# j4n1k/rl4co-slap

Measured on AMD Instinct MI355X. Metric: env-steps/sec (batch×decode) SLAP & TSP-100 at 1/2/4/8 MI355X, higher is better.
Workload: dtype u8+i64+f32

## Files before the change

rl4co_slap_amd/csrc/co_common.hpp:

```cpp
#pragma once

#include <hip/hip_runtime.h>
#include <stdint.h>

#include "../../include/co_env.h"

namespace co {

constexpr int kWave = 64;

__device__ __forceinline__ int lane_id() { return threadIdx.x & (kWave - 1); }
__device__ __forceinline__ int wave_in_block() {
  return __builtin_amdgcn_readfirstlane(threadIdx.x >> 6);
}

template <typename T>
__device__ __forceinline__ T wave_sum(T v) {
#pragma unroll
  for (int off = 32; off > 0; off >>= 1) v += __shfl_xor(v, off, kWave);
  return v;
}

__device__ __forceinline__ float wave_max(float v) {
#pragma unroll
  for (int off = 32; off > 0; off >>= 1) v = fmaxf(v, __shfl_xor(v, off, kWave));
  return v;
}

__device__ __forceinline__ int wave_min_int(int v) {
#pragma unroll
  for (int off = 32; off > 0; off >>= 1) v = min(v, __shfl_xor(v, off, kWave));
  return v;
}

__device__ __forceinline__ bool argmax_better(float a, int ia, float b, int ib) {
  const bool na = a != a, nb = b != b;
  if (na || nb) return na && (!nb || ia < ib);
  return a > b || (a == b && ia < ib);
}

__device__ __forceinline__ void wave_argmax(float& v, int& idx) {
#pragma unroll
  for (int off = 32; off > 0; off >>= 1) {
    const float ov = __shfl_xor(v, off, kWave);
    const int oi = __shfl_xor(idx, off, kWave);
    if (argmax_better(ov, oi, v, idx)) { v = ov; idx = oi; }
  }
}

__device__ __forceinline__ void wave_argmin(float& v, int& idx) {
#pragma unroll
  for (int off = 32; off > 0; off >>= 1) {
    const float ov = __shfl_xor(v, off, kWave);
    const int oi = __shfl_xor(idx, off, kWave);
    if (ov < v || (ov == v && oi < idx)) { v = ov; idx = oi; }
  }
}

__device__ __forceinline__ void set_status(int32_t* status, int32_t bits) {
  if (status) atomicOr(status, bits);
}

__device__ __forceinline__ float edge_len(float x0, float y0, float x1, float y1) {
  const float dx = x1 - x0, dy = y1 - y0;
  return sqrtf(dx * dx + dy * dy);
}

template <int CTRL>
__device__ __forceinline__ uint32_t dpp_u(uint32_t v) {
  return (uint32_t)__builtin_amdgcn_update_dpp(0, (int)v, CTRL, 0xf, 0xf, false);
}

template <int RL, class Take>
__device__ __forceinline__ void grp_reduce2(uint32_t& v, uint32_t& a, Take take) {
  uint32_t ov, oa;
#define CO_DPP_STAGE(C)                      \
  ov = dpp_u<C>(v);                          \
  oa = dpp_u<C>(a);                          \
  if (take(ov, oa, v, a)) { v = ov; a = oa; }
  if (RL >= 2) { CO_DPP_STAGE(0xB1); }
  if (RL >= 4) { CO_DPP_STAGE(0x4E); }
  if (RL >= 8) { CO_DPP_STAGE(0x141); }
  if (RL >= 16) { CO_DPP_STAGE(0x140); }
#undef CO_DPP_STAGE
  if (RL >= 32) {
    const auto rv = __builtin_amdgcn_permlane16_swap(v, v, false, false);
    const auto ra = __builtin_amdgcn_permlane16_swap(a, a, false, false);
    v = rv[0]; a = ra[0];
    if (take(rv[1], ra[1], v, a)) { v = rv[1]; a = ra[1]; }
  }
  if (RL >= 64) {
    const auto rv = __builtin_amdgcn_permlane32_swap(v, v, false, false);
    const auto ra = __builtin_amdgcn_permlane32_swap(a, a, false, false);
    v = rv[0]; a = ra[0];
    if (take(rv[1], ra[1], v, a)) { v = rv[1]; a = ra[1]; }
  }
}

template <int RL, class Op>
__device__ __forceinline__ uint32_t grp_reduce(uint32_t v, Op op) {
  if (RL >= 2) v = op(v, dpp_u<0xB1>(v));
  if (RL >= 4) v = op(v, dpp_u<0x4E>(v));
  if (RL >= 8) v = op(v, dpp_u<0x141>(v));
  if (RL >= 16) v = op(v, dpp_u<0x140>(v));
  if (RL >= 32) {
    const auto r = __builtin_amdgcn_permlane16_swap(v, v, false, false);
    v = op(r[0], r[1]);
  }
  if (RL >= 64) {
    const auto r = __builtin_amdgcn_permlane32_swap(v, v, false, false);
    v = op(r[0], r[1]);
  }
  return v;
}

template <int RL>
__device__ __forceinline__ double grp_sum_f64(double v) {
  uint32_t lo = (uint32_t)__double_as_longlong(v), hi = (uint32_t)(__double_as_longlong(v) >> 32);
  auto join = [](uint32_t l, uint32_t h) {
    return __longlong_as_double((long long)(((uint64_t)h << 32) | l));
  };
#define CO_DPP_F64(C)                                   \
  {                                                     \
    v = v + join(dpp_u<C>(lo), dpp_u<C>(hi));           \
    lo = (uint32_t)__double_as_longlong(v);             \
    hi = (uint32_t)(__double_as_longlong(v) >> 32);     \
  }
  if (RL >= 2) CO_DPP_F64(0xB1);
  if (RL >= 4) CO_DPP_F64(0x4E);
  if (RL >= 8) CO_DPP_F64(0x141);
  if (RL >= 16) CO_DPP_F64(0x140);
#undef CO_DPP_F64
  if (RL >= 32) {
    const auto rl = __builtin_amdgcn_permlane16_swap(lo, lo, false, false);
    const auto rh = __builtin_amdgcn_permlane16_swap(hi, hi, false, false);
    v = join(rl[0], rh[0]) + join(rl[1], rh[1]);
    lo = (uint32_t)__double_as_longlong(v);
    hi = (uint32_t)(__double_as_longlong(v) >> 32);
  }
  if (RL >= 64) {
    const auto rl = __builtin_amdgcn_permlane32_swap(lo, lo, false, false);
    const auto rh = __builtin_amdgcn_permlane32_swap(hi, hi, false, false);
    v = join(rl[0], rh[0]) + join(rl[1], rh[1]);
  }
  return v;
}

template <int RL>
__device__ __forceinline__ float grp_max(float v) {
  return __uint_as_float(grp_reduce<RL>(__float_as_uint(v), [](uint32_t x, uint32_t y) {
    return __float_as_uint(fmaxf(__uint_as_float(x), __uint_as_float(y)));
  }));
}
template <int RL>
__device__ __forceinline__ float grp_max_ord(float v) {
  const int b = __float_as_int(v);
  int o = b ^ ((b >> 31) & 0x7fffffff);
  o = (int)grp_reduce<RL>((uint32_t)o, [](uint32_t x, uint32_t y) {
    return (uint32_t)max((int)x, (int)y);
  });
  return __int_as_float(o ^ ((o >> 31) & 0x7fffffff));
}
template <int RL>
__device__ __forceinline__ float grp_sum(float v) {
  return __uint_as_float(grp_reduce<RL>(__float_as_uint(v), [](uint32_t x, uint32_t y) {
    return __float_as_uint(__uint_as_float(x) + __uint_as_float(y));
  }));
}
template <int RL>
__device__ __forceinline__ void grp_argmax(float& v, int& idx) {
  uint32_t uv = __float_as_uint(v), ui = (uint32_t)idx;
  grp_reduce2<RL>(uv, ui, [](uint32_t ov, uint32_t oi, uint32_t cv, uint32_t ci) {
    return argmax_better(__uint_as_float(ov), (int)oi, __uint_as_float(cv), (int)ci);
  });
  v = __uint_as_float(uv);
  idx = (int)ui;
}
template <int RL>
__device__ __forceinline__ int grp_min_int(int v) {
  return (int)grp_reduce<RL>((uint32_t)v, [](uint32_t x, uint32_t y) {
    return (uint32_t)min((int)x, (int)y);
  });
}
template <int RL>
__device__ __forceinline__ int grp_max_int(int v) {
  return (int)grp_reduce<RL>((uint32_t)v, [](uint32_t x, uint32_t y) {
    return (uint32_t)max((int)x, (int)y);
  });
}

template <int RL>
__device__ __forceinline__ void grp_argmin(float& v, int& idx) {
  uint32_t uv = __float_as_uint(v), ui = (uint32_t)idx;
  grp_reduce2<RL>(uv, ui, [](uint32_t ov, uint32_t oi, uint32_t cv, uint32_t ci) {
    const float a = __uint_as_float(ov), b = __uint_as_float(cv);
    return a < b || (a == b && (int)oi < (int)ci);
  });
  v = __uint_as_float(uv);
  idx = (int)ui;
}

template <int RL>
__device__ __forceinline__ void grp_argmin_split(float& v, int& idx) {
  const float m = __uint_as_float(grp_reduce<RL>(__float_as_uint(v), [](uint32_t a, uint32_t b) {
    return __float_as_uint(fminf(__uint_as_float(a), __uint_as_float(b)));
  }));
  const int cand = v == m ? idx : 0x7fffffff;
  idx = (int)grp_reduce<RL>((uint32_t)cand, [](uint32_t a, uint32_t b) {
    return (uint32_t)min((int)a, (int)b);
  });
  v = m;
}

constexpr uint32_t kDistKeyInf = 0xff800000u;
__device__ __forceinline__ uint32_t dist_key(float d) {
  const uint32_t u = __float_as_uint(d + 0.0f);
  return u ^ ((uint32_t)((int32_t)u >> 31) | 0x80000000u);
}
__device__ __forceinline__ uint32_t key_sel32(uint64_t m, uint32_t t, uint32_t f) {
  uint32_t r;
  asm("v_cndmask_b32_e64 %0, %1, %2, %3" : "=v"(r) : "v"(f), "v"(t), "s"(m));
  return r;
}
__device__ __forceinline__ void key_cswap(uint64_t& a, uint64_t& b) {
  const uint64_t lt = __builtin_amdgcn_ballot_w64(a < b);
  const uint32_t alo = (uint32_t)a, ahi = (uint32_t)(a >> 32), blo = (uint32_t)b,
                 bhi = (uint32_t)(b >> 32);
  a = ((uint64_t)key_sel32(lt, ahi, bhi) << 32) | key_sel32(lt, alo, blo);
  b = ((uint64_t)key_sel32(lt, bhi, ahi) << 32) | key_sel32(lt, blo, alo);
}
template <int E>
__device__ __forceinline__ void sort_keys(uint64_t (&k)[E]) {
  static_assert((E & (E - 1)) == 0, "E must be a power of two");
#pragma unroll
  for (int p = 1; p < E; p <<= 1)
#pragma unroll
    for (int q = p; q > 0; q >>= 1)
#pragma unroll
      for (int j = q % p; j + q < E; j += 2 * q)
#pragma unroll
        for (int i = 0; i < q; ++i)
          if (i + j + q < E && (i + j) / (2 * p) == (i + j + q) / (2 * p))
            key_cswap(k[i + j], k[i + j + q]);
}

typedef __attribute__((address_space(3))) void lds_void;

template <int AUX = 0>
__device__ __forceinline__ void stage_bytes_lds(const unsigned char* __restrict__ src, int nbytes,
                                                unsigned char* dst) {
  const int lane = threadIdx.x & 63, wave = wave_in_block(), nw = blockDim.x >> 6;
  const int n16 = nbytes & ~15;
  for (int base = wave * 1024; base < n16; base += nw * 1024) {
    const int off = base + lane * 16;
    if (off < n16)
      __builtin_amdgcn_global_load_lds((const void*)(src + off), (lds_void*)(dst + base), 16, 0,
                                       AUX);
  }
  for (int k = n16 + (int)threadIdx.x; k < nbytes; k += blockDim.x) dst[k] = src[k];
  __builtin_amdgcn_s_waitcnt(0);
  __syncthreads();
}

template <int AUX = 0>
__device__ __forceinline__ void wave_dma(const unsigned char* __restrict__ src, int nbytes,
                                         unsigned char* dst) {
  const int lane = lane_id(), n16 = nbytes & ~15;
  for (int base = 0; base < n16; base += 1024) {
    if (base + lane * 16 < n16)
      __builtin_amdgcn_global_load_lds((const void*)(src + base + lane * 16),
                                       (lds_void*)(dst + base), 16, 0, AUX);
  }
  if (lane < ((nbytes - n16) >> 2))
    reinterpret_cast<uint32_t*>(dst + n16)[lane] = reinterpret_cast<const uint32_t*>(src + n16)[lane];
}

__device__ __forceinline__ void wave_dma_wait() {
  __builtin_amdgcn_s_waitcnt(0);
  __builtin_amdgcn_fence(__ATOMIC_RELEASE, "wavefront");
  __builtin_amdgcn_wave_barrier();
  __builtin_amdgcn_fence(__ATOMIC_ACQUIRE, "wavefront");
}

namespace {
__global__ void zero_i32_kernel(int32_t* p) { *p = 0; }
}
inline int zero_i32(int32_t* p, hipStream_t s) {
  hipLaunchKernelGGL(zero_i32_kernel, dim3(1), dim3(1), 0, s, p);
  return (int)hipGetLastError();
}

inline unsigned grid_for(int64_t work_items, int per_block, int64_t cap = 256 * 16) {
  int64_t g = (work_items + per_block - 1) / per_block;
  if (g < 1) g = 1;
  if (g > cap) g = cap;
  return (unsigned)g;
}

constexpr int64_t kMaxCoverThreads = ((int64_t)1 << 32) - 1;
inline unsigned cover_grid(int64_t work_items, int per_block, int block_threads = 256) {
  int64_t g = (work_items + per_block - 1) / per_block;
  if (g < 1) g = 1;
  if (g * (int64_t)block_threads > kMaxCoverThreads) return 0;
  return (unsigned)g;
}

inline int launch_status() {
  hipError_t e = hipGetLastError();
  return e == hipSuccess ? CO_OK : (int)e;
}

}

int co_internal_tsp_reward_stepmajor(int64_t B, int64_t N, const float* locs,
                                     int64_t locs_batch, const int64_t* acts, int64_t st,
                                     int check, float* reward, int32_t* status, void* stream);
int co_internal_tsp_reward_rows(int64_t B, int64_t N, const float* locs, int64_t locs_batch,
                                const int64_t* acts, int64_t sb, int check, float* reward,
                                int32_t* status, void* stream);
int co_internal_tsp_nearest_rollout(int64_t B, int64_t N, const float* locs, int64_t* acts_out,
                                    uint8_t* mask_out, int64_t* first_out, int64_t* cur_out,
                                    int64_t* i_out, uint8_t* done_out, uint8_t* step_reward_out,
                                    float* reward_out, void* stream);
```

rl4co_slap_amd/csrc/rollout.hip:

```cpp
#include "co_common.hpp"

using namespace co;

namespace {


inline int NW_launch(int64_t n) {
  const int w = (int)((n + 63) / 64);
  return w <= 1 ? 1 : (w == 2 ? 2 : 4);
}

template <int NW>
__device__ __forceinline__ void mask_row_to_lds(const uint64_t (&m)[NW], int n,
                                                unsigned char* row, int c_lo = 0,
                                                int c_hi = -1) {
  if (c_hi < 0) c_hi = n;
  if ((n & 3) == 0 && (c_lo & 3) == 0) {
    for (int c = c_lo; c < c_hi; c += 4) {
      uint32_t v = 0;
#pragma unroll
      for (int j = 0; j < 4; ++j) {
        const int cc = c + j;
        uint64_t w = 0;
#pragma unroll
        for (int k = 0; k < NW; ++k)
          if ((cc >> 6) == k) w = m[k];
        v |= (uint32_t)((w >> (cc & 63)) & 1ull) << (8 * j);
      }
      *reinterpret_cast<uint32_t*>(row + c) = v;
    }
  } else {
    for (int c = c_lo; c < c_hi; ++c) {
      uint64_t w = 0;
#pragma unroll
      for (int k = 0; k < NW; ++k)
        if ((c >> 6) == k) w = m[k];
      row[c] = (unsigned char)((w >> (c & 63)) & 1ull);
    }
  }
}

__device__ __forceinline__ void copy_tile_out(const unsigned char* scratch, int nbytes,
                                              uint8_t* __restrict__ dst) {
  const int tid = threadIdx.x;
  const int n16 = ((reinterpret_cast<uintptr_t>(dst) & 15) == 0) ? (nbytes & ~15) : 0;
  for (int off = tid * 16; off < n16; off += blockDim.x * 16)
    *reinterpret_cast<uint4*>(dst + off) = *reinterpret_cast<const uint4*>(scratch + off);
  for (int k = n16 + tid; k < nbytes; k += blockDim.x) dst[k] = scratch[k];
}

__device__ __forceinline__ void zero_tile_out(int nbytes, uint8_t* __restrict__ dst) {
  const int tid = threadIdx.x;
  const int n16 = ((reinterpret_cast<uintptr_t>(dst) & 15) == 0) ? (nbytes & ~15) : 0;
  for (int off = tid * 16; off < n16; off += blockDim.x * 16)
    *reinterpret_cast<uint4*>(dst + off) = make_uint4(0u, 0u, 0u, 0u);
  for (int k = n16 + tid; k < nbytes; k += blockDim.x) dst[k] = 0;
}

__host__ __device__ inline size_t tsp_tile_bytes(int N, int Q) {
  const size_t xy = (size_t)64 * N * 8;
  const size_t scr = (((size_t)64 * N + 15) & ~(size_t)15) + (size_t)Q * 64 * 8 + 64 * 8 + 64 * 4 +
                     16 * 4;
  return ((xy > scr ? xy : scr) + 15) & ~(size_t)15;
}

#ifndef CO_TEACH_Q
#define CO_TEACH_Q 4
#endif
#ifndef CO_TEACH_U
#define CO_TEACH_U 8
#endif
template <int NW, int Q, bool STATE, int NB = 0>
__global__ __launch_bounds__(64 * Q) void tsp_teacher_kernel(
    int64_t B, int N, const float2* __restrict__ locs, int64_t LB,
    const int64_t* __restrict__ acts_in, uint8_t* __restrict__ mask_out,
    int64_t* __restrict__ first_out, int64_t* __restrict__ cur_out, int64_t* __restrict__ i_out,
    uint8_t* __restrict__ done_out, uint8_t* __restrict__ step_reward_out,
    float* __restrict__ reward_out, int check, int32_t* status) {
  extern __shared__ __attribute__((aligned(16))) unsigned char smem[];
  float2* s_xy = reinterpret_cast<float2*>(smem);
  constexpr int VS = 2 * NW + 1;
  uint32_t* s_vis = reinterpret_cast<uint32_t*>(smem + tsp_tile_bytes(N, Q));
  const int lane = threadIdx.x & 63, q = wave_in_block();
  const int64_t row0 = (int64_t)blockIdx.x * 64;
  const int rows = (int)((B - row0) < 64 ? (B - row0) : 64);
  const int64_t b = row0 + lane;
  const bool live = lane < rows;

  const int R = (N - 1 + Q - 1) / Q;
  const int t_lo = 1 + q * R < N ? 1 + q * R : N;
  const int t_hi = t_lo + R < N ? t_lo + R : N;
  constexpr int U = CO_TEACH_U;
  int64_t bufA[U], bufB[U];
  const int64_t* ap = acts_in + (live ? b : row0);
  auto load = [&](int64_t (&dst)[U], int t0) {
    const int tc = t0 + U <= t_hi ? t0 : t_hi - U;
    const int64_t* p = ap + (int64_t)tc * B;
#pragma unroll
    for (int u = 0; u < U; ++u) {
      dst[u] = *p;
      p += B;
    }
  };
  const int nfull = (t_hi - t_lo) / U;
  const int64_t a_prev = ap[(int64_t)(q == 0 ? 0 : t_lo - 1) * B];
  if (nfull > 0) load(bufA, t_lo);
  if (q == 0) {
    for (int k = 0; k < NW; ++k) {
      const int lo = k * 64;
      const uint64_t w = (N >= lo + 64) ? ~0ull : (N > lo ? ((1ull << (N - lo)) - 1ull) : 0ull);
      s_vis[lane * VS + 2 * k] = (uint32_t)w;
      s_vis[lane * VS + 2 * k + 1] = (uint32_t)(w >> 32);
    }
  }
  stage_bytes_lds(reinterpret_cast<const unsigned char*>(locs + (row0 % LB) * N), rows * N * 8,
                  reinterpret_cast<unsigned char*>(s_xy));
  const float2* xy = s_xy + lane * N;
  uint32_t* vw = s_vis + lane * VS;
  uint32_t badw = 0;
  int a = 0;
  float px = 0.f, py = 0.f, fx = 0.f, fy = 0.f;
  double len = 0.0;
  if (live) {
    const uint32_t lo = (uint32_t)a_prev;
    const uint32_t in = ((uint32_t)(a_prev >> 32) == 0u) & (lo < (uint32_t)N);
    a = in ? (int)lo : 0;
    if (q == 0) {
      badw |= in ^ 1u;
      __hip_atomic_fetch_and(&vw[a >> 5], ~(1u << (a & 31)), __ATOMIC_RELAXED,
                             __HIP_MEMORY_SCOPE_WORKGROUP);
    }
    const float2 p0 = xy[a];
    px = fx = p0.x;
    py = fy = p0.y;
    auto run = [&](const int64_t (&src)[U], int cnt) {
      int av[U];
#pragma unroll
      for (int u = 0; u < U; ++u) {
        if (u < cnt) {
          const uint32_t l32 = (uint32_t)src[u];
          const uint32_t ok = ((uint32_t)(src[u] >> 32) == 0u) & (l32 < (uint32_t)N);
          badw |= ok ^ 1u;
          av[u] = ok ? (int)l32 : 0;
        }
      }
      float2 qq[U];
#pragma unroll
      for (int u = 0; u < U; ++u)
        if (u < cnt) qq[u] = xy[av[u]];
#pragma unroll
      for (int u = 0; u < U; ++u)
        if (u < cnt)
          __hip_atomic_fetch_and(&vw[av[u] >> 5], ~(1u << (av[u] & 31)), __ATOMIC_RELAXED,
                                 __HIP_MEMORY_SCOPE_WORKGROUP);
      __builtin_amdgcn_sched_barrier(0);
#pragma unroll
      for (int u = 0; u < U; ++u) {
        if (u < cnt) {
          const float ox = u ? qq[u - 1].x : px, oy = u ? qq[u - 1].y : py;
          const float dx = qq[u].x - ox, dy = qq[u].y - oy;
          len += (double)__builtin_amdgcn_sqrtf(dx * dx + dy * dy);
        }
      }
#pragma unroll
      for (int u = 0; u < U; ++u)
        if (u + 1 == cnt) {
          px = qq[u].x;
          py = qq[u].y;
          a = av[u];
        }
    };
    int k = 0;
    for (; k + 1 < nfull; k += 2) {
      load(bufB, t_lo + (k + 1) * U);
      run(bufA, U);
      load(bufA, t_lo + (k + 2) * U);
      run(bufB, U);
    }
    if (k < nfull) run(bufA, U);
    const int tail = t_hi - t_lo - nfull * U;
    if (tail > 0) {
      const int t0 = t_lo + nfull * U;
#pragma unroll
      for (int u = 0; u < U; ++u) bufB[u] = (u < tail) ? ap[(int64_t)(t0 + u) * B] : 0;
      run(bufB, tail);
    }
  }
  if (__any(badw != 0u && check) && lane == 0) set_status(status, CO_ST_INVALID_TOUR);
  __syncthreads();
  const int qlast = N >= 2 ? (N - 2) / R : 0;
  const size_t mbytes = ((size_t)64 * N + 15) & ~(size_t)15;
  double* s_len = reinterpret_cast<double*>(smem + mbytes);
  float2* s_last = reinterpret_cast<float2*>(s_len + Q * 64);
  int* s_lasta = reinterpret_cast<int*>(s_last + 64);
  s_len[q * 64 + lane] = len;
  if (q == qlast) {
    s_last[lane] = make_float2(px, py);
    s_lasta[lane] = a;
  }
  uint64_t m[NW];
#pragma unroll
  for (int kk = 0; kk < NW; ++kk) m[kk] = (uint64_t)vw[2 * kk] | ((uint64_t)vw[2 * kk + 1] << 32);
  bool empty = true;
#pragma unroll
  for (int kk = 0; kk < NW; ++kk) empty &= (m[kk] == 0);
  if (q == 0 && __any(live && !empty && check) && lane == 0)
    set_status(status, CO_ST_INVALID_TOUR);
  int* s_flag = s_lasta + 64;
  bool all_empty = false;
  if (STATE) {
    const bool wave_empty = __ballot(live && !empty) == 0ull;
    if (lane == 0) s_flag[q] = wave_empty;
    __syncthreads();
    all_empty = true;
#pragma unroll
    for (int w = 0; w < Q; ++w) all_empty &= s_flag[w] != 0;
  }
  if (STATE && !all_empty) {
    if (live) {
      const int per = ((N + 4 * Q - 1) / (4 * Q)) * 4;
      const int c_lo = q * per < N ? q * per : N;
      const int c_hi = c_lo + per < N ? c_lo + per : N;
      mask_row_to_lds<NW>(m, N, smem + (size_t)lane * N, c_lo, c_hi);
    }
    __syncthreads();
  } else if (!STATE) {
    __syncthreads();
  }
  if (q == 0 && live) {
    double tot = 0.0;
#pragma unroll
    for (int w = 0; w < Q; ++w) tot += s_len[w * 64 + lane];
    const float2 pl = s_last[lane];
    const int first = ((uint64_t)a_prev < (uint64_t)N) ? (int)a_prev : 0;
    tot += (double)edge_len(pl.x, pl.y, fx, fy);
    reward_out[b] = -(float)tot;
    if (STATE) {
      first_out[b] = first;
      cur_out[b] = s_lasta[lane];
      i_out[b] = N;
      done_out[b] = empty;
      step_reward_out[b] = 0;
    }
  }
  if (STATE) {
    if (all_empty)
      zero_tile_out(rows * N, mask_out + row0 * N);
    else
      copy_tile_out(smem, rows * N, mask_out + row0 * N);
  }
}

#ifndef CO_ROWS_EPL112
#define CO_ROWS_EPL112 7
#endif

__host__ __device__ inline size_t tsp_rows_wave_bytes(int gpw, int N) {
  return ((size_t)gpw * N * 8 + 15) & ~(size_t)15;
}

#ifndef CO_ROWS_WPB
#define CO_ROWS_WPB 4
#endif
template <int G, int EPL, int MODE, bool STATE>
__global__ __launch_bounds__(64 * CO_ROWS_WPB) void tsp_teacher_rows_kernel(
    int64_t B, int N, const float2* __restrict__ locs, int64_t LB,
    const int64_t* __restrict__ acts, int64_t sb, uint8_t* __restrict__ mask_out,
    int64_t* __restrict__ first_out, int64_t* __restrict__ cur_out, int64_t* __restrict__ i_out,
    uint8_t* __restrict__ done_out, uint8_t* __restrict__ step_reward_out,
    float* __restrict__ reward_out, int check, int32_t* status) {
  constexpr int GPW = 64 / G;
  constexpr bool VEC = MODE == 1 && EPL % 2 == 0, DMA = MODE == 3;
  __shared__ uint32_t s_bits[CO_ROWS_WPB][GPW][(G * EPL + 31) / 32];
  extern __shared__ __attribute__((aligned(16))) unsigned char s_rows[];
  constexpr int NWB = (G * EPL + 31) / 32;
  const int lane = lane_id(), sl = lane % G, grp = lane / G, w = wave_in_block();
  uint32_t* bits = s_bits[w][grp];
  unsigned char* s_w = s_rows + (DMA ? (size_t)w * tsp_rows_wave_bytes(GPW, N) : 0);
  const float2* s_xy = reinterpret_cast<const float2*>(s_w);
  const int64_t wid = (int64_t)blockIdx.x * (blockDim.x >> 6) + w;
  const int nwords = (N + 31) >> 5;
  const int t0 = sl * EPL;
  {
    const int64_t base = wid * GPW;
    if (base >= B) return;
    const int64_t r = base + grp;
    const bool valid = r < B;
    const int64_t rr = valid ? r : 0;
    const int64_t* arow = acts + rr * sb;
    if constexpr (DMA) {
      __builtin_amdgcn_s_waitcnt(0xc07f);
      const int rows = (int)(B - base < GPW ? B - base : GPW);
      const int64_t lb = LB == B ? base : base % LB;
      wave_dma<2>(reinterpret_cast<const unsigned char*>(locs + lb * N), rows * N * 8, s_w);
    }
    int64_t av[EPL];
    if constexpr (MODE == 3) {
#pragma unroll
      for (int k = 0; k < EPL; ++k) av[k] = arow[t0 + k < N ? t0 + k : N - 1];
    }
    if constexpr (DMA) wave_dma_wait();
    if constexpr (MODE == 3) {
    } else if constexpr (VEC) {
#pragma unroll
      for (int k = 0; k < EPL; k += 2) {
        if (valid && t0 + k + 1 < N) {
          const longlong2 v = *reinterpret_cast<const longlong2*>(arow + t0 + k);
          av[k] = v.x;
          av[k + 1] = v.y;
        } else {
          av[k] = (valid && t0 + k < N) ? arow[t0 + k] : 0;
          av[k + 1] = 0;
        }
      }
    } else {
#pragma unroll
      for (int k = 0; k < EPL; ++k) av[k] = (valid && t0 + k < N) ? arow[t0 + k] : 0;
    }
    for (int j = sl; j < NWB; j += G) bits[j] = 0u;
    uint32_t bad = 0;
    int node[EPL];
#pragma unroll
    for (int k = 0; k < EPL; ++k) {
      const uint32_t l32 = (uint32_t)av[k];
      const bool ok = ((uint32_t)(av[k] >> 32) == 0u) & (l32 < (uint32_t)N);
      const bool in = t0 + k < N;
      bad |= (in && !ok) ? 1u : 0u;
      node[k] = ok ? (int)l32 : 0;
    }
    const float2* lrow = DMA ? s_xy + grp * N : locs + (LB == B ? rr : rr % LB) * (int64_t)N;
    float2 p[EPL];
    if constexpr (DMA) {
#pragma unroll
      for (int k = 0; k < EPL; ++k) p[k] = lrow[node[k]];
    } else {
#pragma unroll
      for (int k = 0; k < EPL; ++k)
        p[k] = (valid && t0 + k < N) ? lrow[node[k]] : make_float2(0.f, 0.f);
    }
    __builtin_amdgcn_fence(__ATOMIC_RELEASE, "wavefront");
    __builtin_amdgcn_wave_barrier();
    __builtin_amdgcn_fence(__ATOMIC_ACQUIRE, "wavefront");
#pragma unroll
    for (int k = 0; k < EPL; ++k)
      __hip_atomic_fetch_or(&bits[node[k] >> 5],
                            (valid && t0 + k < N) ? 1u << (node[k] & 31) : 0u, __ATOMIC_RELAXED,
                            __HIP_MEMORY_SCOPE_WAVEFRONT);
    double acc = 0.0;
#pragma unroll
    for (int k = 1; k < EPL; ++k) {
      const float dx = p[k].x - p[k - 1].x, dy = p[k].y - p[k - 1].y;
      const float e = __builtin_amdgcn_sqrtf(dx * dx + dy * dy);
      acc += t0 + k < N ? (double)e : 0.0;
    }
    const float nx = __shfl_down(p[0].x, 1, G), ny = __shfl_down(p[0].y, 1, G);
    const float fx = __shfl(p[0].x, 0, G), fy = __shfl(p[0].y, 0, G);
    const int tl = N - 1 - t0;
    float lx = p[EPL - 1].x, ly = p[EPL - 1].y;
#pragma unroll
    for (int k = 0; k < EPL - 1; ++k)
      if (k == tl) {
        lx = p[k].x;
        ly = p[k].y;
      }
    {
      const bool cross = t0 + EPL < N, closing = !cross && tl >= 0 && tl < EPL;
      const float tx = cross ? nx : fx, ty = cross ? ny : fy;
      const float dx = tx - lx, dy = ty - ly;
      const float e = __builtin_amdgcn_sqrtf(dx * dx + dy * dy);
      acc += (cross || closing) ? (double)e : 0.0;
    }
    const float len = (float)grp_sum_f64<G>(acc);
    __builtin_amdgcn_fence(__ATOMIC_RELEASE, "wavefront");
    __builtin_amdgcn_wave_barrier();
    __builtin_amdgcn_fence(__ATOMIC_ACQUIRE, "wavefront");
    int cnt = 0;
    for (int j = sl; j < nwords; j += G) cnt += __popc(bits[j]);
    cnt = (int)grp_reduce<G>((uint32_t)cnt, [](uint32_t x, uint32_t y) { return x + y; });
    bad = grp_reduce<G>(bad, [](uint32_t x, uint32_t y) { return x | y; });
    const bool full = cnt == N;
    if (check && valid && sl == 0 && (bad || !full)) set_status(status, CO_ST_INVALID_TOUR);
    if (!valid) return;
    if constexpr (STATE) {
      uint8_t* mrow = mask_out + r * (int64_t)N;
      const bool wide = ((reinterpret_cast<uintptr_t>(mrow) | (uintptr_t)N) & 3) == 0;
      if (wide) {
        for (int c4 = sl; c4 < (N >> 2); c4 += G) {
          uint32_t v = 0;
          if (!full) {
            const uint32_t nib = ~(bits[c4 >> 3] >> (4 * (c4 & 7))) & 0xfu;
            v = (nib & 1u) | ((nib & 2u) << 7) | ((nib & 4u) << 14) | ((nib & 8u) << 21);
          }
          __builtin_nontemporal_store(v, reinterpret_cast<uint32_t*>(mrow + 4 * c4));
        }
      } else {
        for (int c = sl; c < N; c += G)
          mrow[c] = full ? 0 : (uint8_t)(((bits[c >> 5] >> (c & 31)) & 1u) ^ 1u);
      }
      const int last_lane = (N - 1) / EPL;
      int lastnode = node[0];
#pragma unroll
      for (int k = 0; k < EPL; ++k)
        if (k == tl) lastnode = node[k];
      if (sl == 0) {
        first_out[r] = node[0];
        i_out[r] = N;
        reward_out[r] = -(float)len;
      }
      if (sl == last_lane) cur_out[r] = lastnode;
      if (sl == (G > 2 ? 2 : 1) % G) {
        done_out[r] = full;
        step_reward_out[r] = 0;
      }
    } else {
      if (sl == 0) reward_out[r] = -(float)len;
    }
  }
}

__device__ __forceinline__ float edge_len_hw(float x0, float y0, float x1, float y1) {
  const float dx = x1 - x0, dy = y1 - y0;
  return __builtin_amdgcn_sqrtf(dx * dx + dy * dy);
}
__device__ __forceinline__ int slap_pick_loc(int pp, const int32_t* asg, int L, bool& range) {
  const bool neg = pp < 0;
  int64_t loc = asg[neg ? 0 : pp];
  loc = loc < 0 ? loc + L : loc;
  const bool bad = neg || loc < 0 || loc >= L;
  range |= bad;
  return bad ? 0 : (int)loc;
}
template <int KU, typename PK>
__device__ __forceinline__ float slap_order_len(const PK* pk, const int32_t* asg,
                                                const float2* xy, int L, bool& range,
                                                int K = KU) {
  int pp[KU], lc[KU];
  float2 q[KU];
#pragma unroll
  for (int k = 0; k < KU; ++k) pp[k] = k < K ? pk[k] : 0;
#pragma unroll
  for (int k = 0; k < KU; ++k) lc[k] = k < K ? slap_pick_loc(pp[k], asg, L, range) : 0;
#pragma unroll
  for (int k = 0; k < KU; ++k) q[k] = xy[lc[k]];
  float len = 0.f;
#pragma unroll
  for (int k = 1; k < KU; ++k)
    if (k < K) len += edge_len_hw(q[k - 1].x, q[k - 1].y, q[k].x, q[k].y);
  float2 ql = q[0];
#pragma unroll
  for (int k = 1; k < KU; ++k) ql = (k == K - 1) ? q[k] : ql;
  return len + edge_len_hw(ql.x, ql.y, q[0].x, q[0].y);
}

__host__ __device__ inline size_t slap_asg_bytes(int ipb, int P) {
  return ((size_t)ipb * P * 4 + 15) & ~(size_t)15;
}
__host__ __device__ inline size_t slap_wave_bytes(int gpw, int epl, int L, int O, int K) {
  const size_t keys = (size_t)epl * 64 * 8;
  const size_t data = (size_t)gpw * (L * 8 + O * 4 + O * K * 2);
  return ((keys > data ? keys : data) + 15) & ~(size_t)15;
}
__host__ __device__ inline size_t slap_xy_bytes(int gpw, int L) {
  return ((size_t)gpw * L * 8 + 15) & ~(size_t)15;
}
__host__ __device__ inline size_t slap_wave_bytes_sd(int gpw, int epl, int L, int O, int K) {
  size_t area = (size_t)(epl - 2) * 64 * 8;
  const size_t dd = (size_t)gpw * L * 4, tail = (size_t)gpw * (O * 4 + O * K * 2);
  area = area > dd ? area : dd;
  area = area > tail ? area : tail;
  return slap_xy_bytes(gpw, L) + ((area + 15) & ~(size_t)15);
}

__device__ __forceinline__ float2 ld_pair(const float2* p) { return *p; }

template <int G, int EPL, bool CLOSEST, bool SD>
__global__ __launch_bounds__(256) void slap_group_kernel(
    int64_t B, int L, int P, int O, int K, const float2* __restrict__ locs,
    const int64_t* __restrict__ picklist, const float* __restrict__ depot_dist,
    const int32_t* __restrict__ assign_in, const int64_t* __restrict__ acts_in,
    int64_t* __restrict__ acts_out, uint8_t* __restrict__ mask_out,
    int32_t* __restrict__ assign_out, int64_t* __restrict__ i_out, uint8_t* __restrict__ done_out,
    uint8_t* __restrict__ step_reward_out, float* __restrict__ reward_out,
    float* __restrict__ ratio_out, int32_t* status) {
  constexpr int IPB = 256 / G, GPW = 64 / G;
  extern __shared__ __attribute__((aligned(16))) unsigned char smem[];
  const int lane = lane_id(), sl = lane % G, g = threadIdx.x / G, gw = lane / G;
  int32_t* s_asg = reinterpret_cast<int32_t*>(smem);
  unsigned char* wreg =
      smem + slap_asg_bytes(IPB, P) +
      (size_t)wave_in_block() * (SD ? slap_wave_bytes_sd(GPW, EPL, L, O, K)
                                    : slap_wave_bytes(GPW, EPL, L, O, K));
  unsigned char* area = wreg + (SD ? slap_xy_bytes(GPW, L) : 0);
  uint64_t* s_keys = reinterpret_cast<uint64_t*>(area) - (SD ? 2 * 64 : 0);
  const int64_t b = (int64_t)blockIdx.x * IPB + g;
  const bool live = b < B;
  const int64_t bb = live ? b : 0;
  float2* xy = reinterpret_cast<float2*>(wreg) + gw * L;
  int32_t* asg = s_asg + g * P;
  unsigned char* obase = SD ? area : wreg + (size_t)GPW * L * 8;
  float* olen = reinterpret_cast<float*>(obase) + gw * O;
  int16_t* pks = reinterpret_cast<int16_t*>(obase + (size_t)GPW * O * 4) + gw * O * K;
  const int64_t wbase = (int64_t)blockIdx.x * IPB + (int64_t)wave_in_block() * GPW;
  const int wrows = (int)(B - wbase < GPW ? (B - wbase > 0 ? B - wbase : 0) : GPW);
  if constexpr (SD) {
    wave_dma<2>(reinterpret_cast<const unsigned char*>(depot_dist + wbase * L), wrows * L * 4,
                area);
    wave_dma_wait();
  }

  float dd[EPL];
  uint32_t avail = 0;
#pragma unroll
  for (int k = 0; k < EPL; ++k) {
    const int c = sl + G * k;
    const bool ok = c < L && c != 0;
    if (ok) avail |= 1u << k;
    if constexpr (SD)
      dd[k] = (CLOSEST && ok) ? reinterpret_cast<const float*>(area)[gw * L + c] : __builtin_inff();
    else
      dd[k] = (CLOSEST && ok) ? (depot_dist + bb * L)[c] : __builtin_inff();
  }
  if constexpr (SD) {
    __builtin_amdgcn_s_waitcnt(0xc07f);
    wave_dma<2>(reinterpret_cast<const unsigned char*>(locs + wbase * L), wrows * L * 8, wreg);
  }
  if (live && ratio_out) {
    float* rrow = ratio_out + bb * L;
    if (((reinterpret_cast<uintptr_t>(ratio_out) | ((uintptr_t)L * 4)) & 15) == 0) {
      for (int c4 = sl; c4 < (L >> 2); c4 += G)
        *reinterpret_cast<float4*>(rrow + 4 * c4) = make_float4(0.f, 0.f, 0.f, 0.f);
    } else {
      for (int c = sl; c < L; c += G) rrow[c] = 0.f;
    }
  }
  const float2* lrow = locs + bb * L;
  const int64_t* prow = picklist + bb * (int64_t)O * K;
  float2 xr[EPL];
  int64_t pr[EPL];
#pragma unroll
  for (int k = 0; k < EPL; ++k) {
    const int c = sl + G * k;
    if constexpr (!SD) xr[k] = c < L ? ld_pair(lrow + c) : make_float2(0.f, 0.f);
    pr[k] = c < O * K ? prow[c] : 0;
  }
  auto wrap_product = [&](int64_t pp) -> int32_t {
    if (pp < 0) pp += P;
    return (pp < 0 || pp >= P) ? -1 : (int32_t)pp;
  };
  int32_t pw[EPL];
#pragma unroll
  for (int k = 0; k < EPL; ++k) pw[k] = wrap_product(pr[k]);
  uint64_t key[EPL];
  if (CLOSEST) {
#pragma unroll
    for (int k = 0; k < EPL; ++k)
      key[k] = ((uint64_t)dist_key(dd[k]) << 32) | (uint32_t)(sl + G * k);
    sort_keys<EPL>(key);
  }
  bool range = false;
  if (CLOSEST) {
    uint64_t hk = key[0], nk = EPL > 1 ? key[1] : ~0ull;
#pragma unroll
    for (int k = 2; k < EPL; ++k) s_keys[k * 64 + lane] = key[k];
    int h = 2;
    for (int t = 0; t < P; ++t) {
      const uint32_t hh = (uint32_t)(hk >> 32);
      const uint32_t gm = grp_reduce<G>(hh, [](uint32_t x, uint32_t y) { return x < y ? x : y; });
      const uint32_t cand = hh == gm ? (uint32_t)hk : 0xffffffffu;
      const uint32_t gi =
          grp_reduce<G>(cand, [](uint32_t x, uint32_t y) { return x < y ? x : y; });
      const bool any = gm < kDistKeyInf;
      if (any && (uint32_t)hk == gi) {
        avail &= ~(1u << (gi / G));
        hk = nk;
        nk = h < EPL ? s_keys[h * 64 + lane] : ~0ull;
        ++h;
      }
      if (sl == 0) asg[t] = any ? (int32_t)gi : 0;
    }
  } else {
    int32_t* s_w = reinterpret_cast<int32_t*>(wreg) + gw * P;
    if (P * GPW <= EPL * 128) {
#pragma unroll 4
      for (int t = sl; t < P; t += G) {
        const int64_t a64 = acts_in[(int64_t)t * B + bb];
        asg[t] = (int32_t)a64;
        const int64_t a = a64 < 0 ? a64 + L : a64;
        const bool bad = a < 0 || a >= L;
        range |= bad;
        s_w[t] = bad ? -1 : (int)a;
      }
      __builtin_amdgcn_fence(__ATOMIC_RELEASE, "wavefront");
      __builtin_amdgcn_wave_barrier();
      __builtin_amdgcn_fence(__ATOMIC_ACQUIRE, "wavefront");
      for (int t = 0; t < P; ++t) {
        const int a = s_w[t];
        if (a >= 0 && sl == a % G) avail &= ~(1u << (a / G));
      }
    } else {
      for (int t = 0; t < P; ++t) {
        const int64_t a64 = acts_in[(int64_t)t * B + bb];
        if (sl == 0) asg[t] = (int32_t)a64;
        const int64_t a = a64 < 0 ? a64 + L : a64;
        if (a < 0 || a >= L) {
          range = true;
        } else if (sl == (int)(a % G)) {
          avail &= ~(1u << (int)(a / G));
        }
      }
    }
  }
  if constexpr (SD) {
    __builtin_amdgcn_s_waitcnt(0);
  } else {
#pragma unroll
    for (int k = 0; k < EPL; ++k) {
      const int c = sl + G * k;
      if (c < L) xy[c] = xr[k];
    }
  }
#pragma unroll
  for (int k = 0; k < EPL; ++k) {
    const int c = sl + G * k;
    if (c < O * K) pks[c] = (int16_t)pw[k];
  }
  for (int c = sl + G * EPL; c < O * K; c += G) pks[c] = (int16_t)wrap_product(prow[c]);
  __builtin_amdgcn_fence(__ATOMIC_RELEASE, "wavefront");
  __builtin_amdgcn_wave_barrier();
  __builtin_amdgcn_fence(__ATOMIC_ACQUIRE, "wavefront");

  if (CLOSEST) {
    constexpr int IPW = 64 / G;
    const int w0 = wave_in_block() * IPW;
    for (int idx = lane; idx < IPW * P; idx += 64) {
      const int t = idx / IPW, gi = idx - t * IPW;
      const int64_t be = (int64_t)blockIdx.x * IPB + w0 + gi;
      if (be < B) {
        int64_t* dst = acts_out + (int64_t)t * B + be;
        *dst = (int64_t)s_asg[(w0 + gi) * P + t];
      }
    }
  }
  for (int o = sl; o < O; o += G) {
    const int16_t* pk = pks + o * K;
    float len = 0.f;
    if (K == 5) {
      len = slap_order_len<5>(pk, asg, xy, L, range);
    } else if (K <= 8) {
      len = slap_order_len<8>(pk, asg, xy, L, range, K);
    } else {
      float2 p0 = make_float2(0.f, 0.f), prev = p0;
      for (int k = 0; k < K; ++k) {
        const float2 q = xy[slap_pick_loc(pk[k], asg, L, range)];
        if (k == 0) {
          p0 = q;
        } else {
          len += edge_len_hw(prev.x, prev.y, q.x, q.y);
        }
        prev = q;
      }
      len += edge_len_hw(prev.x, prev.y, p0.x, p0.y);
    }
    olen[o] = len;
  }
  __builtin_amdgcn_fence(__ATOMIC_RELEASE, "wavefront");
  __builtin_amdgcn_wave_barrier();
  __builtin_amdgcn_fence(__ATOMIC_ACQUIRE, "wavefront");

  if (live) {
    uint8_t* mrow = mask_out + bb * L;
    if (((reinterpret_cast<uintptr_t>(mask_out) | (uintptr_t)L) & 3) == 0) {
      uint8_t* sm = reinterpret_cast<uint8_t*>(xy);
#pragma unroll
      for (int k = 0; k < EPL; ++k) {
        const int c = sl + G * k;
        if (c < L) sm[c] = (uint8_t)((avail >> k) & 1u);
      }
      __builtin_amdgcn_fence(__ATOMIC_RELEASE, "wavefront");
      __builtin_amdgcn_wave_barrier();
      __builtin_amdgcn_fence(__ATOMIC_ACQUIRE, "wavefront");
      for (int d = sl; d < (L >> 2); d += G)
        *reinterpret_cast<uint32_t*>(mrow + 4 * d) = *reinterpret_cast<const uint32_t*>(sm + 4 * d);
    } else {
#pragma unroll
      for (int k = 0; k < EPL; ++k) {
        const int c = sl + G * k;
        if (c < L) {
          uint8_t* dst = mrow + c;
          *dst = (uint8_t)((avail >> k) & 1u);
        }
      }
    }
    if (((reinterpret_cast<uintptr_t>(assign_out) | ((uintptr_t)P * 4)) & 15) == 0) {
      for (int c4 = sl; c4 < (P >> 2); c4 += G)
        *reinterpret_cast<int4*>(assign_out + bb * P + 4 * c4) =
            *reinterpret_cast<const int4*>(asg + 4 * c4);
    } else {
#pragma unroll 2
      for (int c = sl; c < P; c += G) {
        int32_t* dst = assign_out + bb * P + c;
        *dst = asg[c];
      }
    }
    if (sl == 0) {
      float total = 0.f;
      int o = 0;
      if ((O & 3) == 0 && (reinterpret_cast<uintptr_t>(olen) & 15) == 0)
        for (; o < O; o += 4) {
          const float4 v = *reinterpret_cast<const float4*>(olen + o);
          total += -v.x;
          total += -v.y;
          total += -v.z;
          total += -v.w;
        }
      for (; o < O; ++o) total += -olen[o];
      reward_out[bb] = total;
      i_out[bb] = P;
      done_out[bb] = 1;
      step_reward_out[bb] = 0;
    }
  }
  if (__any(range && live) && lane == 0) set_status(status, CO_ST_INDEX_RANGE);
}


template <bool STATE>
int launch_tsp_teacher(int64_t B, int64_t N, const float2* l2, int64_t LB, const int64_t* acts,
                       uint8_t* mask_out, int64_t* first_out, int64_t* cur_out, int64_t* i_out,
                       uint8_t* done_out, uint8_t* step_reward_out, float* reward_out, int check,
                       int32_t* status, hipStream_t s) {
  constexpr int Q = CO_TEACH_Q;
  const int NW = NW_launch(N);
  const size_t shmem = tsp_tile_bytes((int)N, Q) + (size_t)64 * (2 * NW + 1) * 4;
  const dim3 grid(cover_grid(B, 64, 64 * Q)), block(64 * Q);
  if (grid.x == 0) return CO_E_INVAL;
#define CO_TEACH(W)                                                                            \
  do {                                                                                         \
    if (shmem > 64 * 1024)                                                                     \
      (void)hipFuncSetAttribute((const void*)tsp_teacher_kernel<W, Q, STATE, 0>,               \
                                hipFuncAttributeMaxDynamicSharedMemorySize, (int)shmem);       \
    hipLaunchKernelGGL((tsp_teacher_kernel<W, Q, STATE, 0>), grid, block, shmem, s, B, (int)N, \
                       l2, LB, acts, mask_out, first_out, cur_out, i_out, done_out,                \
                       step_reward_out, reward_out, check, status);                            \
  } while (0)
  if (NW == 1) CO_TEACH(1);
  else if (NW == 2) CO_TEACH(2);
  else CO_TEACH(4);
#undef CO_TEACH
  return launch_status();
}

template <bool STATE>
int launch_tsp_rows(int64_t B, int64_t N, const float2* l2, int64_t LB, const int64_t* acts,
                    int64_t sb, uint8_t* mask_out, int64_t* first_out, int64_t* cur_out,
                    int64_t* i_out, uint8_t* done_out, uint8_t* step_reward_out,
                    float* reward_out, int check, int32_t* status, hipStream_t s) {
  const bool vec = ((reinterpret_cast<uintptr_t>(acts) & 15) == 0) && (sb % 2 == 0);
  const bool dma_ok = sb == N &&
                      ((reinterpret_cast<uintptr_t>(acts) | reinterpret_cast<uintptr_t>(l2)) & 15) == 0;
#define CO_ROWS(GG, EE)                                                                        \
  do {                                                                                         \
    constexpr int WPB = CO_ROWS_WPB;                                                           \
    const dim3 grid(cover_grid((B + 64 / GG - 1) / (64 / GG), WPB, 64 * WPB)), block(64 * WPB); \
    if (grid.x == 0) return CO_E_INVAL;                                                        \
    const size_t dsh = WPB * tsp_rows_wave_bytes(64 / GG, (int)N);                             \
           \
    const size_t sbits = (size_t)WPB * (64 / GG) * ((GG * EE + 31) / 32) * 4;                  \
    if (dma_ok && (LB == B || LB % (64 / GG) == 0) && dsh + sbits <= 64 * 1024)                \
      hipLaunchKernelGGL((tsp_teacher_rows_kernel<GG, EE, 3, STATE>), grid, block, dsh, s, B,   \
                         (int)N, l2, LB, acts, sb, mask_out, first_out, cur_out, i_out,        \
                         done_out, step_reward_out, reward_out, check, status);                \
    else if (vec)                                                                              \
      hipLaunchKernelGGL((tsp_teacher_rows_kernel<GG, EE, 1, STATE>), grid, block, 0, s, B,     \
                         (int)N, l2, LB, acts, sb, mask_out, first_out, cur_out, i_out,        \
                         done_out, step_reward_out, reward_out, check, status);                \
    else                                                                                       \
      hipLaunchKernelGGL((tsp_teacher_rows_kernel<GG, EE, 0, STATE>), grid, block, 0, s, B,     \
                         (int)N, l2, LB, acts, sb, mask_out, first_out, cur_out, i_out,        \
                         done_out, step_reward_out, reward_out, check, status);                \
  } while (0)
  if (N <= 32) CO_ROWS(4, 8);
  else if (N <= 64) CO_ROWS(8, 8);
  else if (N <= 16 * CO_ROWS_EPL112) CO_ROWS(16, CO_ROWS_EPL112);
  else if (N <= 128) CO_ROWS(16, 8);
  else if (N <= 256) CO_ROWS(32, 8);
  else if (N <= 512) CO_ROWS(64, 8);
  else CO_ROWS(64, 16);
#undef CO_ROWS
  return launch_status();
}

}

int co_internal_tsp_reward_rows(int64_t B, int64_t N, const float* locs, int64_t locs_batch,
                                const int64_t* acts, int64_t sb, int check, float* reward,
                                int32_t* status, void* stream) {
  if (N > 1024 || sb < N || (reinterpret_cast<uintptr_t>(locs) & 7)) return CO_E_INVAL;
  return launch_tsp_rows<false>(B, N, reinterpret_cast<const float2*>(locs), locs_batch, acts, sb,
                                nullptr, nullptr, nullptr, nullptr, nullptr, nullptr, reward,
                                check, status, (hipStream_t)stream);
}

namespace {
int tsp_rollout_stepwise(int64_t B, int64_t N, const float* locs, const int64_t* acts_in,
                         int64_t* acts_out, uint8_t* mask_out, int64_t* first_out,
                         int64_t* cur_out, int64_t* i_out, uint8_t* done_out,
                         uint8_t* step_reward_out, float* reward_out, int check, int32_t* status,
                         void* stream) {
  int rc = co_tsp_reset(B, N, mask_out, first_out, cur_out, i_out, reward_out, stream);
  const bool nearest = acts_in == nullptr;
  const int64_t* acts = nearest ? acts_out : acts_in;
  for (int64_t t = 0; t < N && rc == CO_OK; ++t) {
    if (nearest)
      rc = co_tsp_nearest_action(B, N, locs, mask_out, cur_out, t == 0, acts_out + t * B,
                                 stream);
    if (rc == CO_OK)
      rc = co_tsp_step(B, N, acts + t * B, mask_out, mask_out, i_out, i_out, first_out,
                       first_out, cur_out, done_out, step_reward_out, t == 0 ? 1 : 0, nullptr,
                       status, stream);
  }
  if (rc != CO_OK) return rc;
  return co_tsp_reward(B, N, N, locs, B, acts, 1, B, check, reward_out, status, stream);
}
}

extern "C" int co_tsp_rollout_ex(int64_t B, int64_t N, const float* locs,
                                 const int64_t* acts_in, int64_t sb, int64_t st,
                                 int64_t* acts_out, uint8_t* mask_out, int64_t* first_out,
                                 int64_t* cur_out, int64_t* i_out, uint8_t* done_out,
                                 uint8_t* step_reward_out, float* reward_out, int check,
                                 int32_t* status, void* stream) {
  if (B < 0 || N <= 0 || N > (1 << 24)) return CO_E_INVAL;
  if (B == 0) return CO_OK;
  const bool nearest = acts_in == nullptr;
  if (!locs || !mask_out || !first_out || !cur_out || !i_out || !done_out || !step_reward_out ||
      !reward_out || (nearest && !acts_out) || (check && !status))
    return CO_E_INVAL;
  if (reinterpret_cast<uintptr_t>(locs) & 7) return CO_E_ALIGN;
  if (!nearest && !(sb == 1 && st == B)) {
    if (st != 1 || sb < N || N > 1024) return CO_E_INVAL;
    return launch_tsp_rows<true>(B, N, reinterpret_cast<const float2*>(locs), B, acts_in, sb,
                                 mask_out, first_out, cur_out, i_out, done_out, step_reward_out,
                                 reward_out, check, status, (hipStream_t)stream);
  }
  if (N > (nearest ? 1024 : 256))
    return tsp_rollout_stepwise(B, N, locs, acts_in, acts_out, mask_out, first_out, cur_out,
                                i_out, done_out, step_reward_out, reward_out, check, status,
                                stream);
  if (nearest)
    return co_internal_tsp_nearest_rollout(B, N, locs, acts_out, mask_out, first_out, cur_out,
                                           i_out, done_out, step_reward_out, reward_out, stream);
  if (reinterpret_cast<uintptr_t>(locs) & 15) return CO_E_ALIGN;
  return launch_tsp_teacher<true>(B, N, reinterpret_cast<const float2*>(locs), B, acts_in,
                                  mask_out,
                                  first_out, cur_out, i_out, done_out, step_reward_out,
                                  reward_out, check, status, (hipStream_t)stream);
}

extern "C" int co_tsp_rollout(int64_t B, int64_t N, const float* locs, const int64_t* acts_in,
                              int64_t* acts_out, uint8_t* mask_out, int64_t* first_out,
                              int64_t* cur_out, int64_t* i_out, uint8_t* done_out,
                              uint8_t* step_reward_out, float* reward_out, int check,
                              int32_t* status, void* stream) {
  return co_tsp_rollout_ex(B, N, locs, acts_in, 1, B, acts_out, mask_out, first_out, cur_out,
                           i_out, done_out, step_reward_out, reward_out, check, status, stream);
}

int co_internal_tsp_reward_stepmajor(int64_t B, int64_t N, const float* locs,
                                     int64_t locs_batch, const int64_t* acts, int64_t st,
                                     int check, float* reward, int32_t* status, void* stream) {
  if (st != B || N > 256 || (reinterpret_cast<uintptr_t>(locs) & 15)) return CO_E_INVAL;
  if (locs_batch != B && locs_batch % 64 != 0) return CO_E_INVAL;
  return launch_tsp_teacher<false>(B, N, reinterpret_cast<const float2*>(locs), locs_batch, acts,
                                   nullptr,
                                   nullptr, nullptr, nullptr, nullptr, nullptr, reward, check,
                                   status, (hipStream_t)stream);
}

extern "C" int co_slap_rollout(int64_t B, int64_t L, int64_t P, int64_t O, int64_t K,
                               const float* locs, const int64_t* picklist,
                               const float* depot_dist, const int32_t* assign_in,
                               const int64_t* acts_in, int64_t* acts_out, uint8_t* mask_out,
                               int32_t* assign_out, int64_t* i_out, uint8_t* done_out,
                               uint8_t* step_reward_out, float* reward_out, float* ratio_out,
                               int32_t* status, void* stream) {
  if (B < 0 || L <= 1 || L > 256 || P <= 0 || O <= 0 || K <= 0 || P > 4096) return CO_E_INVAL;
  if (B == 0) return CO_OK;
  const bool closest = acts_in == nullptr;
  if (!locs || !picklist || !assign_in || !mask_out || !assign_out || !i_out || !done_out ||
      !step_reward_out || !reward_out || !status || (closest && (!acts_out || !depot_dist)))
    return CO_E_INVAL;
  if (reinterpret_cast<uintptr_t>(locs) & 7) return CO_E_ALIGN;
  const int G = L <= 64 ? 8 : (L <= 128 ? 16 : 32);
  const int ipb = 256 / G;
  const bool sd = closest && (L % 4) == 0 &&
                  ((reinterpret_cast<uintptr_t>(locs) | reinterpret_cast<uintptr_t>(depot_dist)) &
                   15) == 0;
  const size_t shmem =
      slap_asg_bytes(ipb, (int)P) +
      4 * (sd ? slap_wave_bytes_sd(64 / G, 8, (int)L, (int)O, (int)K)
              : slap_wave_bytes(64 / G, 8, (int)L, (int)O, (int)K));
  if (shmem > 160 * 1024) return CO_E_INVAL;
  const dim3 grid(cover_grid(B, ipb)), block(256);
  if (grid.x == 0) return CO_E_INVAL;
  hipStream_t s = (hipStream_t)stream;
  const float2* l2 = reinterpret_cast<const float2*>(locs);
#define CO_SLAP(GG, EPL, C, SDD)                                                               \
  do {                                                                                         \
    if (shmem > 64 * 1024)                                                                     \
      (void)hipFuncSetAttribute((const void*)slap_group_kernel<GG, EPL, C, SDD>,               \
                                hipFuncAttributeMaxDynamicSharedMemorySize, (int)shmem);       \
    hipLaunchKernelGGL((slap_group_kernel<GG, EPL, C, SDD>), grid, block, shmem, s, B, (int)L, \
                       (int)P, (int)O, (int)K, l2, picklist, depot_dist, assign_in, acts_in,   \
                       acts_out, mask_out, assign_out, i_out, done_out, step_reward_out,       \
                       reward_out, ratio_out, status);                                         \
  } while (0)
#define CO_SLAP_G(C, SDD)                                       \
  if (G == 8) CO_SLAP(8, 8, C, SDD);                            \
  else if (G == 16) CO_SLAP(16, 8, C, SDD);                     \
  else CO_SLAP(32, 8, C, SDD)
  if (closest && sd) {
    CO_SLAP_G(true, true);
  } else if (closest) {
    CO_SLAP_G(true, false);
  } else {
    CO_SLAP_G(false, false);
  }
#undef CO_SLAP_G
#undef CO_SLAP
  return launch_status();
}
```

Baseline: 353.0 billion.

## Switch SLAP rollout to blocked per-lane location layout with ballot-based argmin

Locations are now owned in contiguous blocks per lane (c = lane*EPL + k) instead of strided by group size. This lets depot distances be read as float4 quads from LDS and mask bytes be packed and stored directly as uint32 without an LDS staging round-trip and barrier. The greedy closest-assignment loop replaces the second group min-reduction with a ballot plus lowest-lane selection, and the winning lane writes asg itself. It adds a static requirement that EPL be a multiple of 4 and a power of two, and clamps tail quad reads to L-4.

```diff
diff --git a/rl4co_slap_amd/csrc/co_common.hpp b/rl4co_slap_amd/csrc/co_common.hpp
--- a/rl4co_slap_amd/csrc/co_common.hpp
+++ b/rl4co_slap_amd/csrc/co_common.hpp
@@ -115,6 +115,13 @@
 }
 
 template <int RL>
+__device__ __forceinline__ uint64_t grp_lowest_lane(uint64_t m) {
+  static_assert(RL >= 2 && RL <= 64 && (RL & (RL - 1)) == 0, "RL must be a power of two");
+  constexpr uint64_t ones = RL == 64 ? 1ull : ~0ull / ((1ull << (RL & 63)) - 1);
+  return m & ~(m - ones);
+}
+
+template <int RL>
 __device__ __forceinline__ double grp_sum_f64(double v) {
   uint32_t lo = (uint32_t)__double_as_longlong(v), hi = (uint32_t)(__double_as_longlong(v) >> 32);
   auto join = [](uint32_t l, uint32_t h) {
diff --git a/rl4co_slap_amd/csrc/rollout.hip b/rl4co_slap_amd/csrc/rollout.hip
--- a/rl4co_slap_amd/csrc/rollout.hip
+++ b/rl4co_slap_amd/csrc/rollout.hip
@@ -510,13 +510,26 @@
 
   float dd[EPL];
   uint32_t avail = 0;
+  if constexpr (SD) {
+    static_assert(EPL % 4 == 0, "a lane's locations are read as quads");
+    const float* drow = reinterpret_cast<const float*>(area) + gw * L;
+#pragma unroll
+    for (int q = 0; q < EPL / 4; ++q) {
+      const int c0 = sl * EPL + 4 * q;
+      const float4 v = *reinterpret_cast<const float4*>(drow + (c0 < L ? c0 : L - 4));
+      dd[4 * q] = v.x;
+      dd[4 * q + 1] = v.y;
+      dd[4 * q + 2] = v.z;
+      dd[4 * q + 3] = v.w;
+    }
+  }
 #pragma unroll
   for (int k = 0; k < EPL; ++k) {
-    const int c = sl + G * k;
+    const int c = sl * EPL + k;
     const bool ok = c < L && c != 0;
     if (ok) avail |= 1u << k;
     if constexpr (SD)
-      dd[k] = (CLOSEST && ok) ? reinterpret_cast<const float*>(area)[gw * L + c] : __builtin_inff();
+      dd[k] = (CLOSEST && ok) ? dd[k] : __builtin_inff();
     else
       dd[k] = (CLOSEST && ok) ? (depot_dist + bb * L)[c] : __builtin_inff();
   }
@@ -554,29 +567,33 @@
   if (CLOSEST) {
 #pragma unroll
     for (int k = 0; k < EPL; ++k)
-      key[k] = ((uint64_t)dist_key(dd[k]) << 32) | (uint32_t)(sl + G * k);
+      key[k] = ((uint64_t)dist_key(dd[k]) << 32) | (uint32_t)(sl * EPL + k);
     sort_keys<EPL>(key);
   }
   bool range = false;
   if (CLOSEST) {
+    static_assert((EPL & (EPL - 1)) == 0, "slot = location % EPL is a mask");
+    int h = 2;
+    for (int t = sl; t < P; t += G) asg[t] = 0;
     uint64_t hk = key[0], nk = EPL > 1 ? key[1] : ~0ull;
 #pragma unroll
     for (int k = 2; k < EPL; ++k) s_keys[k * 64 + lane] = key[k];
-    int h = 2;
+    __builtin_amdgcn_fence(__ATOMIC_RELEASE, "wavefront");
+    __builtin_amdgcn_wave_barrier();
+    __builtin_amdgcn_fence(__ATOMIC_ACQUIRE, "wavefront");
     for (int t = 0; t < P; ++t) {
       const uint32_t hh = (uint32_t)(hk >> 32);
       const uint32_t gm = grp_reduce<G>(hh, [](uint32_t x, uint32_t y) { return x < y ? x : y; });
-      const uint32_t cand = hh == gm ? (uint32_t)hk : 0xffffffffu;
-      const uint32_t gi =
-          grp_reduce<G>(cand, [](uint32_t x, uint32_t y) { return x < y ? x : y; });
-      const bool any = gm < kDistKeyInf;
-      if (any && (uint32_t)hk == gi) {
-        avail &= ~(1u << (gi / G));
+      const uint64_t own = grp_lowest_lane<G>(__builtin_amdgcn_ballot_w64(hh == gm)) &
+                           __builtin_amdgcn_ballot_w64(hh < kDistKeyInf);
+      if (__builtin_amdgcn_inverse_ballot_w64(own)) {
+        const uint32_t c = (uint32_t)hk;
+        asg[t] = (int32_t)c;
+        avail &= ~(1u << (c & (EPL - 1)));
         hk = nk;
         nk = h < EPL ? s_keys[h * 64 + lane] : ~0ull;
         ++h;
       }
-      if (sl == 0) asg[t] = any ? (int32_t)gi : 0;
     }
   } else {
     int32_t* s_w = reinterpret_cast<int32_t*>(wreg) + gw * P;
@@ -595,7 +612,7 @@
       __builtin_amdgcn_fence(__ATOMIC_ACQUIRE, "wavefront");
       for (int t = 0; t < P; ++t) {
         const int a = s_w[t];
-        if (a >= 0 && sl == a % G) avail &= ~(1u << (a / G));
+        if (a >= 0 && sl == a / EPL) avail &= ~(1u << (a % EPL));
       }
     } else {
       for (int t = 0; t < P; ++t) {
@@ -604,8 +621,8 @@
         const int64_t a = a64 < 0 ? a64 + L : a64;
         if (a < 0 || a >= L) {
           range = true;
-        } else if (sl == (int)(a % G)) {
-          avail &= ~(1u << (int)(a / G));
+        } else if (sl == (int)(a / EPL)) {
+          avail &= ~(1u << (int)(a % EPL));
         }
       }
     }
@@ -670,21 +687,17 @@
   if (live) {
     uint8_t* mrow = mask_out + bb * L;
     if (((reinterpret_cast<uintptr_t>(mask_out) | (uintptr_t)L) & 3) == 0) {
-      uint8_t* sm = reinterpret_cast<uint8_t*>(xy);
+#pragma unroll
+      for (int q = 0; q < EPL / 4; ++q) {
+        const int c0 = sl * EPL + 4 * q;
+        const uint32_t nib = (avail >> (4 * q)) & 0xfu;
+        const uint32_t v = (nib & 1u) | ((nib & 2u) << 7) | ((nib & 4u) << 14) | ((nib & 8u) << 21);
+        if (c0 < L) *reinterpret_cast<uint32_t*>(mrow + c0) = v;
+      }
+    } else {
 #pragma unroll
       for (int k = 0; k < EPL; ++k) {
-        const int c = sl + G * k;
-        if (c < L) sm[c] = (uint8_t)((avail >> k) & 1u);
-      }
-      __builtin_amdgcn_fence(__ATOMIC_RELEASE, "wavefront");
-      __builtin_amdgcn_wave_barrier();
-      __builtin_amdgcn_fence(__ATOMIC_ACQUIRE, "wavefront");
-      for (int d = sl; d < (L >> 2); d += G)
-        *reinterpret_cast<uint32_t*>(mrow + 4 * d) = *reinterpret_cast<const uint32_t*>(sm + 4 * d);
-    } else {
-#pragma unroll
-      for (int k = 0; k < EPL; ++k) {
-        const int c = sl + G * k;
+        const int c = sl * EPL + k;
         if (c < L) {
           uint8_t* dst = mrow + c;
           *dst = (uint8_t)((avail >> k) & 1u);
```

Result: no change. 352.6 billion (median of 2 runs) (-0.1%).
